# BigCiLeng/bilateral-driving

Hardware: AMD Instinct MI355X
Metric: train iters/sec (fwd+bwd) at 2M Gaussians, 6x1920x1080; HBM roofline % (higher is better)
Workload: dtype f32

## Files before the change

### bilateral_driving_amd/csrc/tiles.hip

```cpp
#include "bds_common.h"
#include "gs_math.h"
#include "scan.h"

namespace bds {

constexpr int kScanBlock = 256;
constexpr int kScanItems = 8;
constexpr int kScanTile = kScanBlock * kScanItems;

__global__ __launch_bounds__(kScanBlock) void scan_reduce_kernel(const uint32_t *__restrict__ in, int64_t n,
                                                                uint32_t *__restrict__ block_sums) {
  __shared__ uint32_t lw[kScanBlock / kWave + 1];
  const int64_t base = (int64_t)blockIdx.x * kScanTile + (int64_t)threadIdx.x * kScanItems;
  uint32_t s = 0;
#pragma unroll
  for (int i = 0; i < kScanItems; i++)
    if (base + i < n) s += in[base + i];
  uint32_t tot;
  block_excl_scan(s, tot, lw);
  if (threadIdx.x == 0) block_sums[blockIdx.x] = tot;
}

__global__ __launch_bounds__(kScanBlock) void scan_small_kernel(uint32_t *__restrict__ data, int64_t n,
                                                               uint64_t *__restrict__ total_out) {
// ... 9 lines not shown
  uint32_t tot;
  uint32_t ex = block_excl_scan(s, tot, lw);
#pragma unroll
  for (int i = 0; i < kScanItems; i++) {
    if (base + i < n) data[base + i] = ex;
    ex += v[i];
  }
  if (total_out && threadIdx.x == 0) *total_out = tot;
}

template <bool kSelfOffset>
__global__ __launch_bounds__(kScanBlock) void scan_apply_kernel(const uint32_t *__restrict__ in, int64_t n,
                                                               const uint32_t *__restrict__ block_offsets,
                                                               uint32_t *__restrict__ out, uint64_t *__restrict__ total_out) {
  __shared__ uint32_t lw[kScanBlock / kWave + 1];
  uint32_t my_offset;
  if (kSelfOffset) {
    uint32_t part = 0;
    for (int b = threadIdx.x; b < (int)blockIdx.x; b += kScanBlock) part += block_offsets[b];
    uint32_t tot;
    block_excl_scan(part, tot, lw);
    my_offset = tot;
  } else {
    my_offset = block_offsets[blockIdx.x];
  }
  const int64_t base = (int64_t)blockIdx.x * kScanTile + (int64_t)threadIdx.x * kScanItems;
  uint32_t v[kScanItems];
  uint32_t s = 0;
#pragma unroll
  for (int i = 0; i < kScanItems; i++) {
    v[i] = base + i < n ? in[base + i] : 0u;
    s += v[i];
  }
  uint32_t tot;
  uint32_t ex = block_excl_scan(s, tot, lw) + my_offset;
#pragma unroll
  for (int i = 0; i < kScanItems; i++) {
    if (base + i < n) out[base + i] = ex;
    ex += v[i];
  }
  if (kSelfOffset && total_out && blockIdx.x == gridDim.x - 1 && threadIdx.x == 0) *total_out = (uint64_t)my_offset + tot;
}

static size_t scan_temp_elems(int64_t n) {
  size_t tot = 0;
  while (n > kScanTile) {
    n = cdiv(n, kScanTile);
    tot += align_up((size_t)n, 4);
  }
  return tot + 4;
}

static int exclusive_scan_u32(const uint32_t *in, uint32_t *out, int64_t n, uint32_t *temp, uint64_t *total_out,
                              hipStream_t st) {
  if (n <= kScanTile) {
    if (in != out) {
      if (hipMemcpyAsync(out, in, sizeof(uint32_t) * n, hipMemcpyDeviceToDevice, st) != hipSuccess) return BDS_ELAUNCH;
    }
    hipLaunchKernelGGL(scan_small_kernel, dim3(1), dim3(kScanBlock), 0, st, out, n, total_out);
    BDS_LAUNCH_CHECK();
    return BDS_OK;
  }
  const int64_t nb = cdiv(n, kScanTile);
  uint32_t *sums = temp;
  hipLaunchKernelGGL(scan_reduce_kernel, dim3((unsigned)nb), dim3(kScanBlock), 0, st, in, n, sums);
  BDS_LAUNCH_CHECK();
  if (nb <= 4096) {
    hipLaunchKernelGGL((scan_apply_kernel<true>), dim3((unsigned)nb), dim3(kScanBlock), 0, st, in, n, sums, out, total_out);
    BDS_LAUNCH_CHECK();
    return BDS_OK;
  }
  int rc = exclusive_scan_u32(sums, sums, nb, temp + align_up((size_t)nb, 4), total_out, st);
  if (rc != BDS_OK) return rc;
  hipLaunchKernelGGL((scan_apply_kernel<false>), dim3((unsigned)nb), dim3(kScanBlock), 0, st, in, n, sums, out, nullptr);
  BDS_LAUNCH_CHECK();
  return BDS_OK;
}

constexpr int kSortBlock = 256;
constexpr int kSortRounds = 16;
constexpr int kSortChunk = kSortBlock * kSortRounds;
constexpr int kSortWaves = kSortBlock / kWave;
constexpr int kGroupShift = 6;

template <int kBins, int kRounds>
__device__ __forceinline__ void chunk_hist(uint32_t *h, const uint32_t *__restrict__ keys, int64_t base, int64_t n, int shift,
                                           uint32_t mask) {
  for (int d = threadIdx.x; d < kBins; d += kSortBlock) h[d] = 0;
  __syncthreads();
#pragma unroll 4
  for (int r = 0; r < kRounds; r++) {
    const int64_t i = base + r * kSortBlock + threadIdx.x;
    if (i < n) atomicAdd(&h[(keys[i] >> shift) & mask], 1u);
  }
  __syncthreads();
}

template <int kRounds, bool kVals>
__device__ __forceinline__ void load_and_count(uint32_t *k, uint32_t *v, const uint32_t *__restrict__ keys_in,
                                               const uint32_t *__restrict__ vals_in, int64_t wbase, int64_t n, int shift, uint32_t mask,
                                               uint32_t *wrow) {
  const int lane = threadIdx.x & (kWave - 1);
#pragma unroll
  for (int r = 0; r < kRounds; r++) {
    const int64_t i = wbase + r * kWave + lane;
    k[r] = 0xFFFFFFFFu;
    if (kVals) v[r] = 0;
    if (i < n) {
      k[r] = keys_in[i];
      if (kVals) v[r] = vals_in[i];
      atomicAdd(&wrow[(k[r] >> shift) & mask], 1u);
    }
  }
}

template <int kBins>
__device__ __forceinline__ void counts_to_positions(uint32_t (&wrun)[kSortWaves][kBins], int d, uint32_t base) {
#pragma unroll
  for (int w = 0; w < kSortWaves; w++) {
    const uint32_t c = wrun[w][d];
    wrun[w][d] = base;
    base += c;
  }
}

template <int kBits = 0>
__device__ __forceinline__ uint32_t rank_round(uint32_t d, bool on, uint32_t *wrow, int bits = kBits) {
  const int lane = threadIdx.x & (kWave - 1);
  const unsigned long long lt = lane == 0 ? 0ull : (~0ull >> (64 - lane));
  unsigned long long peers = __ballot(on);
  auto match_bit = [&](int b) {
    const unsigned long long bal = __ballot((d >> b) & 1u);
    peers &= ((d >> b) & 1u) ? bal : ~bal;
  };
  if constexpr (kBits > 0) {
#pragma unroll
    for (int b = 0; b < kBits; b++) match_bit(b);
  } else {
    for (int b = 0; b < bits; b++) match_bit(b);
  }
  const uint32_t rank = __popcll(peers & lt);
  uint32_t pos = 0;
  if (on) pos = wrow[d];
  __builtin_amdgcn_s_waitcnt(0xc07f);
  __builtin_amdgcn_wave_barrier();
  if (on && rank == 0) wrow[d] = pos + __popcll(peers);
  __builtin_amdgcn_wave_barrier();
  return pos + rank;
}

template <int kPer, int kSums>
__device__ __forceinline__ void grouped_bases(const uint32_t *__restrict__ hist, const uint32_t *__restrict__ ghist, int vb, int nb,
                                              uint32_t (&total)[kPer], uint32_t (&below)[kPer]) {
  constexpr int kBins = kSortBlock * kPer;
  const int ng = (nb + (1 << kGroupShift) - 1) >> kGroupShift, gb = vb >> kGroupShift;
#pragma unroll
  for (int u = 0; u < kPer; u++) { total[u] = 0; below[u] = 0; }
  const uint32_t *gp = ghist + threadIdx.x * kPer;
  int g = 0;
  for (; g + 4 <= ng; g += 4) {
    uint32_t c[4][kPer];
#pragma unroll
    for (int j = 0; j < 4; j++)
#pragma unroll
      for (int u = 0; u < kPer; u++) c[j][u] = gp[(int64_t)(g + j) * kBins + u];
#pragma unroll
    for (int u = 0; u < kPer; u++) {
      total[u] += (c[0][u] + c[1][u]) + (c[2][u] + c[3][u]);
      below[u] += (g < gb ? c[0][u] : 0u) + (g + 1 < gb ? c[1][u] : 0u) + (g + 2 < gb ? c[2][u] : 0u) + (g + 3 < gb ? c[3][u] : 0u);
    }
  }
  for (; g < ng; g++) {
#pragma unroll
    for (int u = 0; u < kPer; u++) {
      const uint32_t c = gp[(int64_t)g * kBins + u];
      total[u] += c;
      if (g < gb) below[u] += c;
    }
  }
  const uint32_t *hp = hist + ((int64_t)gb << kGroupShift) * kBins + threadIdx.x * kPer;
  const int nrows = vb - (gb << kGroupShift);
  uint32_t p[kSums][kPer];
#pragma unroll
  for (int j = 0; j < kSums; j++)
#pragma unroll
    for (int u = 0; u < kPer; u++) p[j][u] = 0;
  int r = 0;
  for (; r + kSums <= nrows; r += kSums) {
    uint32_t a[kSums][kPer];
#pragma unroll
    for (int j = 0; j < kSums; j++)
#pragma unroll
      for (int u = 0; u < kPer; u++) a[j][u] = hp[(int64_t)(r + j) * kBins + u];
#pragma unroll
    for (int j = 0; j < kSums; j++)
#pragma unroll
      for (int u = 0; u < kPer; u++) p[j][u] += a[j][u];
  }
  for (; r < nrows; r++) {
#pragma unroll
    for (int u = 0; u < kPer; u++) p[0][u] += hp[(int64_t)r * kBins + u];
  }
#pragma unroll
  for (int u = 0; u < kPer; u++) {
#pragma unroll
    for (int j = 1; j < kSums; j++) p[0][u] += p[j][u];
    below[u] += p[0][u];
  }
}

template <bool kPairs>
__device__ __forceinline__ void write_out_ordered(const uint32_t *lk, const uint32_t *lv, int cnt, int shift, uint32_t mask,
                                                  const uint32_t *gbase, const uint32_t *dstart, uint32_t *__restrict__ keys_out,
                                                  uint32_t *__restrict__ vals_out, const uint32_t *__restrict__ unpack,
                                                  uint32_t rank_mask) {
  for (int i = threadIdx.x; i < cnt; i += kSortBlock) {
    const uint32_t kk = lk[i];
    const uint32_t d = (kk >> shift) & mask;
    const uint32_t g = gbase[d] + ((uint32_t)i - dstart[d]);
    keys_out[g] = kk;
    if (kPairs) vals_out[g] = lv[i];
    else if (unpack) vals_out[g] = unpack[kk & rank_mask];
  }
}
__device__ __forceinline__ int chunk_count(int64_t n, int64_t bbase) {
  return (int)((n - bbase) < (int64_t)kSortChunk ? (n - bbase) : (int64_t)kSortChunk);
}

__global__ __launch_bounds__(kSortBlock) void radix_hist_kernel(const uint32_t *__restrict__ keys, int64_t n_host,
                                                               const uint64_t *__restrict__ n_dev, int shift,
                                                               uint32_t mask, int nblocks,
                                                               uint32_t *__restrict__ hist ) {
  __shared__ uint32_t h[256];
  chunk_hist<256, kSortRounds>(h, keys, (int64_t)blockIdx.x * kSortChunk, list_length(n_host, n_dev), shift, mask);
  if (threadIdx.x <= mask) hist[(int64_t)threadIdx.x * nblocks + blockIdx.x] = h[threadIdx.x];
}

__global__ __launch_bounds__(kSortBlock) void radix_scatter_lds_kernel(
    const uint32_t *__restrict__ keys_in, const uint32_t *__restrict__ vals_in, int64_t n_host,
    const uint64_t *__restrict__ n_dev, int shift, uint32_t mask, int bits, int nblocks,
    const uint32_t *__restrict__ hist_scanned, uint32_t *__restrict__ keys_out, uint32_t *__restrict__ vals_out) {
  const int64_t n = list_length(n_host, n_dev);
  const int64_t bbase = (int64_t)blockIdx.x * kSortChunk;
  if (bbase >= n) return;
  __shared__ uint32_t wrun[kSortWaves][256];
  __shared__ uint32_t dstart[256], gbase[256];
  __shared__ uint32_t lw[kSortBlock / kWave + 1];
  __shared__ uint32_t lk[kSortChunk], lv[kSortChunk];
  const int tid = threadIdx.x, wv = tid / kWave;
#pragma unroll
  for (int w = 0; w < kSortWaves; w++) wrun[w][tid] = 0;
  __syncthreads();
  const int64_t wbase = bbase + (int64_t)wv * (kSortChunk / kSortWaves);
  uint32_t k[kSortRounds], v[kSortRounds];
  load_and_count<kSortRounds, true>(k, v, keys_in, vals_in, wbase, n, shift, mask, wrun[wv]);
  __syncthreads();
  {
    uint32_t tot = 0;
#pragma unroll
    for (int w = 0; w < kSortWaves; w++) tot += wrun[w][tid];
    uint32_t all;
    const uint32_t base = block_excl_scan(tot, all, lw);
    dstart[tid] = base;
    gbase[tid] = tid <= (int)mask ? hist_scanned[(int64_t)tid * nblocks + blockIdx.x] : 0u;
    counts_to_positions(wrun, tid, base);
  }
  __syncthreads();
#pragma unroll
  for (int r = 0; r < kSortRounds; r++) {
    const bool on = wbase + r * kWave + (tid & (kWave - 1)) < n;
    const uint32_t slot = rank_round((k[r] >> shift) & mask, on, wrun[wv], bits);
    if (on) { lk[slot] = k[r]; lv[slot] = v[r]; }
  }
  __syncthreads();
  write_out_ordered<true>(lk, lv, chunk_count(n, bbase), shift, mask, gbase, dstart, keys_out, vals_out, nullptr, 0u);
}

__global__ __launch_bounds__(kSortBlock) void radix_scatter_keys_kernel(
    const uint32_t *__restrict__ keys_in, int64_t n_host, const uint64_t *__restrict__ n_dev, int shift, uint32_t mask, int bits,
    int nblocks, const uint32_t *__restrict__ hist_scanned, uint32_t *__restrict__ keys_out, const uint32_t *__restrict__ unpack,
    uint32_t rank_mask, uint32_t *__restrict__ vals_out) {
  const int64_t n = list_length(n_host, n_dev);
  const int64_t bbase = (int64_t)blockIdx.x * kSortChunk;
  if (bbase >= n) return;
  __shared__ uint32_t wrun[kSortWaves][256];
  __shared__ uint32_t dstart[256], gbase[256];
  __shared__ uint32_t lw[kSortBlock / kWave + 1];
  __shared__ uint32_t lk[kSortChunk];
  const int tid = threadIdx.x, wv = tid / kWave;
#pragma unroll
  for (int w = 0; w < kSortWaves; w++) wrun[w][tid] = 0;
  __syncthreads();
  const int64_t wbase = bbase + (int64_t)wv * (kSortChunk / kSortWaves);
  uint32_t k[kSortRounds];
  load_and_count<kSortRounds, false>(k, nullptr, keys_in, nullptr, wbase, n, shift, mask, wrun[wv]);
  __syncthreads();
  {
    uint32_t tot = 0;
#pragma unroll
    for (int w = 0; w < kSortWaves; w++) tot += wrun[w][tid];
    uint32_t all;
    const uint32_t base = block_excl_scan(tot, all, lw);
    dstart[tid] = base;
    gbase[tid] = tid <= (int)mask ? hist_scanned[(int64_t)tid * nblocks + blockIdx.x] : 0u;
    counts_to_positions(wrun, tid, base);
  }
  __syncthreads();
#pragma unroll
  for (int r = 0; r < kSortRounds; r++) {
    const bool on = wbase + r * kWave + (tid & (kWave - 1)) < n;
    const uint32_t slot = rank_round((k[r] >> shift) & mask, on, wrun[wv], bits);
    if (on) lk[slot] = k[r];
  }
  __syncthreads();
  write_out_ordered<false>(lk, nullptr, chunk_count(n, bbase), shift, mask, gbase, dstart, keys_out, vals_out, unpack, rank_mask);
}

template <int kBins>
__global__ __launch_bounds__(kSortBlock) void radix_hist_wide_kernel(const uint32_t *__restrict__ keys, int64_t n_host,
                                                                    const uint64_t *__restrict__ n_dev, int shift, uint32_t mask,
                                                                    uint32_t *__restrict__ hist ,
                                                                    uint32_t *__restrict__ ghist ) {
  __shared__ uint32_t h[kBins];
  const int64_t n = list_length(n_host, n_dev), base = (int64_t)blockIdx.x * kSortChunk;
  if (base >= n) return;
  chunk_hist<kBins, kSortRounds>(h, keys, base, n, shift, mask);
  for (int d = threadIdx.x; d < kBins; d += kSortBlock) {
    const uint32_t c = h[d];
    hist[(int64_t)blockIdx.x * kBins + d] = c;
    if (c) atomicAdd(&ghist[(int64_t)(blockIdx.x >> kGroupShift) * kBins + d], c);
  }
}

template <int kBins>
__global__ __launch_bounds__(kSortBlock) void radix_scatter_keys_wide_kernel(
    const uint32_t *__restrict__ keys_in, int64_t n_host, const uint64_t *__restrict__ n_dev, int shift, uint32_t mask, int bits,
    const uint32_t *__restrict__ hist, const uint32_t *__restrict__ ghist, uint32_t *__restrict__ keys_out,
    const uint32_t *__restrict__ unpack, uint32_t rank_mask, uint32_t *__restrict__ vals_out, int32_t *__restrict__ offsets_out,
    int n_offsets) {
  constexpr int kPer = kBins / kSortBlock;
  const int64_t n = list_length(n_host, n_dev);
  const int vb = (int)blockIdx.x;
  const int64_t bbase = (int64_t)vb * kSortChunk;
  if (bbase >= n && !(offsets_out && vb == 0)) return;
  __shared__ uint32_t wrun[kSortWaves][kBins];
  __shared__ uint32_t dstart[kBins], gbase[kBins];
  __shared__ uint32_t lw[kSortBlock / kWave + 1];
  __shared__ uint32_t lk[kSortChunk];
  const int tid = threadIdx.x, wv = tid / kWave;
  for (int d = tid; d < kBins; d += kSortBlock) {
#pragma unroll
    for (int w = 0; w < kSortWaves; w++) wrun[w][d] = 0;
  }
  __syncthreads();
  const int64_t wbase = bbase + (int64_t)wv * (kSortChunk / kSortWaves);
  uint32_t k[kSortRounds];
  load_and_count<kSortRounds, false>(k, nullptr, keys_in, nullptr, wbase, n, shift, mask, wrun[wv]);
  __syncthreads();
  {
    uint32_t tot[kPer], sum = 0;
#pragma unroll
    for (int u = 0; u < kPer; u++) {
      const int d = tid * kPer + u;
      tot[u] = 0;
#pragma unroll
      for (int w = 0; w < kSortWaves; w++) tot[u] += wrun[w][d];
      sum += tot[u];
    }
    uint32_t gt[kPer], below[kPer];
    grouped_bases<kPer, 4>(hist, ghist, vb, (int)((n + kSortChunk - 1) / kSortChunk), gt, below);
    uint32_t gsum = 0;
#pragma unroll
    for (int u = 0; u < kPer; u++) gsum += gt[u];
    uint32_t all;
    uint32_t dbase = block_excl_scan(gsum, all, lw);
    uint32_t base = block_excl_scan(sum, all, lw);
#pragma unroll
    for (int u = 0; u < kPer; u++) {
      const int d = tid * kPer + u;
      dstart[d] = base;
      gbase[d] = dbase + below[u];
      dbase += gt[u];
      if (offsets_out && vb == 0 && d < n_offsets) offsets_out[d] = (int32_t)gbase[d];
      counts_to_positions(wrun, d, base);
      base += tot[u];
    }
  }
  __syncthreads();
#pragma unroll
  for (int r = 0; r < kSortRounds; r++) {
    const bool on = wbase + r * kWave + (tid & (kWave - 1)) < n;
    const uint32_t slot = rank_round((k[r] >> shift) & mask, on, wrun[wv], bits);
    if (on) lk[slot] = k[r];
  }
  __syncthreads();
  write_out_ordered<false>(lk, nullptr, chunk_count(n, bbase), shift, mask, gbase, dstart, keys_out, vals_out, unpack, rank_mask);
}

constexpr int kWideBits = 10;

static size_t radix_temp_elems(int64_t n, int max_bins = 256) {
  const int64_t nblocks = cdiv(n > 0 ? n : 1, kSortChunk);
  const size_t h = align_up((size_t)max_bins * nblocks, 4);
  const size_t group_rows = max_bins > 256 ? (size_t)max_bins * (size_t)cdiv(nblocks, 1 << kGroupShift) : 0;
  const size_t behind = scan_temp_elems((int64_t)max_bins * nblocks);
  return h + (behind > group_rows ? behind : group_rows);
}

static size_t radix_wide_group_elems(int64_t n, int bits) {
  return (size_t)(1 << bits) * (size_t)cdiv(cdiv(n > 0 ? n : 1, kSortChunk), 1 << kGroupShift);
}

static int radix_pass(const uint32_t *kin, const uint32_t *vin, uint32_t *kout, uint32_t *vout, int64_t n, int shift,
                      int bits, uint32_t *temp, hipStream_t st, const uint64_t *n_dev = nullptr) {
  if (n == 0) return BDS_OK;
  const int nblocks = (int)cdiv(n, kSortChunk);
  const uint32_t mask = (1u << bits) - 1u;
  const int64_t hn = (int64_t)(mask + 1) * nblocks;
  uint32_t *hist = temp;
  uint32_t *stemp = temp + align_up((size_t)256 * nblocks, 4);
  hipLaunchKernelGGL(radix_hist_kernel, dim3(nblocks), dim3(kSortBlock), 0, st, kin, n, n_dev, shift, mask, nblocks, hist);
  BDS_LAUNCH_CHECK();
  int rc = exclusive_scan_u32(hist, hist, hn, stemp, nullptr, st);
  if (rc != BDS_OK) return rc;
  hipLaunchKernelGGL(radix_scatter_lds_kernel, dim3(nblocks), dim3(kSortBlock), 0, st, kin, vin, n, n_dev, shift, mask, bits,
                     nblocks, hist, kout, vout);
  BDS_LAUNCH_CHECK();
  return BDS_OK;
}


static int radix_pass_keys(const uint32_t *kin, uint32_t *kout, int64_t n, int shift, int bits, uint32_t *temp, hipStream_t st,
                           const uint32_t *unpack, uint32_t rank_mask, uint32_t *vout, int32_t *offsets_out = nullptr,
                           int n_offsets = 0, const uint64_t *n_dev = nullptr) {
  if (n == 0) return BDS_OK;
  const int nblocks = (int)cdiv(n, kSortChunk);
  const uint32_t mask = (1u << bits) - 1u;
  const int64_t hn = (int64_t)(mask + 1) * nblocks;
  uint32_t *hist = temp;
  uint32_t *stemp = temp + align_up((size_t)(bits > 8 ? (1 << kWideBits) : 256) * nblocks, 4);
  if (bits > 8) {
    uint32_t *ghist = stemp;
    if (bits == 9) {
      hipLaunchKernelGGL((radix_hist_wide_kernel<512>), dim3(nblocks), dim3(kSortBlock), 0, st, kin, n, n_dev, shift, mask, hist, ghist);
      hipLaunchKernelGGL((radix_scatter_keys_wide_kernel<512>), dim3(nblocks), dim3(kSortBlock), 0, st, kin, n, n_dev, shift, mask, bits,
                         hist, ghist, kout, unpack, rank_mask, vout, offsets_out, n_offsets);
    } else {
      hipLaunchKernelGGL((radix_hist_wide_kernel<1024>), dim3(nblocks), dim3(kSortBlock), 0, st, kin, n, n_dev, shift, mask, hist, ghist);
      hipLaunchKernelGGL((radix_scatter_keys_wide_kernel<1024>), dim3(nblocks), dim3(kSortBlock), 0, st, kin, n, n_dev, shift, mask, bits,
                         hist, ghist, kout, unpack, rank_mask, vout, offsets_out, n_offsets);
    }
    BDS_LAUNCH_CHECK();
    return BDS_OK;
  }
  hipLaunchKernelGGL(radix_hist_kernel, dim3(nblocks), dim3(kSortBlock), 0, st, kin, n, n_dev, shift, mask, nblocks, hist);
  BDS_LAUNCH_CHECK();
  int rc = exclusive_scan_u32(hist, hist, hn, stemp, nullptr, st);
  if (rc != BDS_OK) return rc;
  hipLaunchKernelGGL(radix_scatter_keys_kernel, dim3(nblocks), dim3(kSortBlock), 0, st, kin, n, n_dev, shift, mask, bits, nblocks,
                     hist, kout, unpack, rank_mask, vout);
  BDS_LAUNCH_CHECK();
  return BDS_OK;
}

constexpr int kShortRounds = 4;
constexpr int kShortChunk = kSortBlock * kShortRounds;
constexpr int kChunkShift = 10;
static_assert(kShortChunk == (1 << kChunkShift), "chunk shift");
constexpr int64_t kShortSortMax = (int64_t)kShortChunk * 8192;

__device__ __forceinline__ int64_t bounded_count(const uint64_t *n_dev, int64_t n_cap) {
  const int64_t n = (int64_t)*n_dev;
  return (n_cap >= 0 && n > n_cap) ? 0 : n;
}
__global__ __launch_bounds__(kSortBlock) void short_hist_kernel(const uint32_t *__restrict__ keys,
                                                               const uint64_t *__restrict__ n_dev, int64_t n_cap, int shift,
                                                               uint32_t *__restrict__ hist ,
                                                               uint32_t *__restrict__ ghist ) {
  __shared__ uint32_t h[256];
  const int64_t n = bounded_count(n_dev, n_cap), base = (int64_t)blockIdx.x * kShortChunk;
  if (base >= n) return;
  chunk_hist<256, kShortRounds>(h, keys, base, n, shift, 255u);
  const uint32_t c = h[threadIdx.x];
  hist[(int64_t)blockIdx.x * 256 + threadIdx.x] = c;
  if (c) atomicAdd(&ghist[(int64_t)(blockIdx.x >> kGroupShift) * 256 + threadIdx.x], c);
}

__global__ __launch_bounds__(kSortBlock) void short_scatter_kernel(
    const uint32_t *__restrict__ keys_in, const uint32_t *__restrict__ vals_in, const uint64_t *__restrict__ n_dev, int64_t n_cap,
    int shift, const uint32_t *__restrict__ hist, const uint32_t *__restrict__ ghist, uint32_t *__restrict__ keys_out,
    uint32_t *__restrict__ vals_out) {
  const int64_t n = bounded_count(n_dev, n_cap);
  const int vb = (int)blockIdx.x;
  if ((int64_t)vb * kShortChunk >= n) return;
  __shared__ uint32_t wrun[kSortWaves][256];
  __shared__ uint32_t lw[kSortBlock / kWave + 1];
  const int tid = threadIdx.x, wv = tid / kWave;
#pragma unroll
  for (int w = 0; w < kSortWaves; w++) wrun[w][tid] = 0;
  uint32_t total[1], below[1];
  grouped_bases<1, 8>(hist, ghist, vb, (int)((n + kShortChunk - 1) >> kChunkShift), total, below);
  uint32_t all;
  const uint32_t digit_base = block_excl_scan(total[0], all, lw);
  const int64_t wbase = (int64_t)vb * kShortChunk + (int64_t)wv * (kShortChunk / kSortWaves);
  uint32_t k[kShortRounds], v[kShortRounds];
  load_and_count<kShortRounds, true>(k, v, keys_in, vals_in, wbase, n, shift, 255u, wrun[wv]);
  __syncthreads();
  counts_to_positions(wrun, tid, digit_base + below[0]);
  __syncthreads();
#pragma unroll
  for (int r = 0; r < kShortRounds; r++) {
    const bool on = wbase + r * kWave + (tid & (kWave - 1)) < n;
    const uint32_t slot = rank_round<8>((k[r] >> shift) & 255u, on, wrun[wv]);
    if (on) {
      keys_out[slot] = k[r];
      vals_out[slot] = v[r];
    }
  }
}

static size_t short_sort_elems(int64_t n_bound) {
  const int64_t nb = cdiv(n_bound > 0 ? n_bound : 1, kShortChunk), ng = cdiv(nb, 1 << kGroupShift);
  return (size_t)(nb + 4 * ng) * 256;
}

constexpr int kIsectBlock = 256;

__global__ __launch_bounds__(kIsectBlock) void isect_flag_kernel(int64_t CN, const int32_t *__restrict__ radii,
                                                                uint32_t *__restrict__ flags) {
  const int64_t o = (int64_t)blockIdx.x * kIsectBlock + threadIdx.x;
  if (o < CN) flags[o] = radii[o] > 0 ? 1u : 0u;
}

__global__ __launch_bounds__(kIsectBlock) void isect_compact_kernel(int64_t CN, const int32_t *__restrict__ radii,
                                                                   const uint32_t *__restrict__ pos,
                                                                   const float *__restrict__ depths,
                                                                   uint32_t *__restrict__ keys, uint32_t *__restrict__ vals,
                                                                   uint32_t *__restrict__ asc, int compact, int sd) {
  const int64_t o = (int64_t)blockIdx.x * kIsectBlock + threadIdx.x;
  if (o >= CN || radii[o] <= 0) return;
  const uint32_t j = pos[o];
  keys[j] = __float_as_uint(depths[o * sd]);
  vals[j] = compact ? j : (uint32_t)o;
  asc[j] = (uint32_t)o;
}

__global__ __launch_bounds__(kScanBlock) void visible_reduce_kernel(int64_t CN, const int32_t *__restrict__ radii,
                                                                   uint32_t *__restrict__ tile_sums,
                                                                   uint32_t *__restrict__ zero_me, int64_t zero_elems,
                                                                   uint64_t *__restrict__ m_total, int32_t *__restrict__ zero_cn) {
  __shared__ uint32_t lw[kScanBlock / kWave + 1];
  if (blockIdx.x == 0 && threadIdx.x == 0) *m_total = 0;
  for (int64_t i = (int64_t)blockIdx.x * kScanBlock + threadIdx.x; i < zero_elems; i += (int64_t)gridDim.x * kScanBlock)
    zero_me[i] = 0u;
  const int64_t base = (int64_t)blockIdx.x * kScanTile + (int64_t)threadIdx.x * kScanItems;
  uint32_t s = 0;
#pragma unroll
  for (int i = 0; i < kScanItems; i++) {
    if (base + i < CN) {
      s += radii[base + i] > 0 ? 1u : 0u;
      if (zero_cn) zero_cn[base + i] = 0;
    }
  }
  uint32_t tot;
  block_excl_scan(s, tot, lw);
  if (threadIdx.x == 0) tile_sums[blockIdx.x] = tot;
}

constexpr int kCompactSpan = kScanTile / kShortChunk + 1;
__global__ __launch_bounds__(kScanBlock) void visible_compact_kernel(int64_t CN, const int32_t *__restrict__ radii,
                                                                    const float *__restrict__ depths,
                                                                    const uint32_t *__restrict__ tile_sums,
                                                                    uint32_t *__restrict__ keys, uint32_t *__restrict__ vals,
                                                                    uint32_t *__restrict__ hist, uint32_t *__restrict__ ghist,
                                                                    uint64_t *__restrict__ n_vis_out, uint32_t *__restrict__ asc,
                                                                    int compact, int sums_per_tile, int sd) {
  constexpr int kSpan = kCompactSpan;
  __shared__ uint32_t lw[kScanBlock / kWave + 1];
  __shared__ uint32_t h[kSpan][256];
  const int vb = (int)blockIdx.x, nvb = (int)gridDim.x;
  uint32_t part = 0;
  for (int b = threadIdx.x; b < vb * sums_per_tile; b += kScanBlock) part += tile_sums[b];
  uint32_t my_offset;
  block_excl_scan(part, my_offset, lw);
  const uint32_t per_sum = (uint32_t)(kScanTile / sums_per_tile);
  const int n_sums = (int)(((uint32_t)CN + per_sum - 1u) / per_sum);
  uint32_t own = 0;
  for (int k = 0; k < sums_per_tile; k++) {
    const int b = vb * sums_per_tile + k;
    if (b < n_sums) own += tile_sums[b];
  }
  if (own == 0) {
    if (vb == nvb - 1 && threadIdx.x == 0) *n_vis_out = (uint64_t)my_offset;
    return;
  }
#pragma unroll
  for (int t = 0; t < kSpan; t++) h[t][threadIdx.x] = 0;
  const int64_t base = (int64_t)vb * kScanTile + (int64_t)threadIdx.x * kScanItems;
  bool vis[kScanItems];
  uint32_t s = 0;
#pragma unroll
  for (int i = 0; i < kScanItems; i++) {
    vis[i] = base + i < CN && radii[base + i] > 0;
    s += vis[i] ? 1u : 0u;
  }
  uint32_t tot;
  uint32_t j = block_excl_scan(s, tot, lw) + my_offset;
  const uint32_t chunk0 = my_offset >> kChunkShift;
#pragma unroll
  for (int i = 0; i < kScanItems; i++) {
    if (vis[i]) {
      const uint32_t key = __float_as_uint(depths[(base + i) * sd]);
      keys[j] = key;
      vals[j] = compact ? j : (uint32_t)(base + i);
      asc[j] = (uint32_t)(base + i);
      atomicAdd(&h[(j >> kChunkShift) - chunk0][key & 255u], 1u);
      j++;
    }
  }
  __syncthreads();
#pragma unroll
  for (int t = 0; t < kSpan; t++) {
    const uint32_t c = h[t][threadIdx.x];
    if (c) {
      atomicAdd(&hist[(int64_t)(chunk0 + t) * 256 + threadIdx.x], c);
      atomicAdd(&ghist[(int64_t)((chunk0 + t) >> kGroupShift) * 256 + threadIdx.x], c);
    }
  }
  if (vb == nvb - 1 && threadIdx.x == 0) *n_vis_out = (uint64_t)my_offset + tot;
}

struct RowStage {
  float mx[kIsectBlock], my[kIsectBlock], a[kIsectBlock], b[kIsectBlock], c[kIsectBlock], qmax[kIsectBlock];
  int x0[kIsectBlock], x1[kIsectBlock], y0[kIsectBlock];
  uint32_t id[kIsectBlock];
  uint32_t cam_base[kIsectBlock];
  uint32_t rowoff[kIsectBlock + 1];
  uint32_t lw[kIsectBlock / kWave + 1];
};

constexpr int kRecWords = 12;

__device__ __forceinline__ uint32_t stage_rows(RowStage &S, int64_t j0, int64_t n_vis, int64_t N, const uint32_t *__restrict__ sorted_idx,
                                               const uint32_t *__restrict__ asc ,
                                               const float *__restrict__ means2d, const int32_t *__restrict__ radii,
                                               const float *__restrict__ conics, const float *__restrict__ opacities,
                                               int tile_size, int tile_w, int tile_h, float4 *__restrict__ rec_out,
                                               const float4 *__restrict__ rec_in, const ProjLayout pl) {
  const int t = threadIdx.x;
  const int64_t j = j0 + t;
  uint32_t nrows = 0;
  if (j < n_vis) {
    if (rec_in != nullptr) {
      const float4 r0 = rec_in[j * 3], r1 = rec_in[j * 3 + 1], r2 = rec_in[j * 3 + 2];
      nrows = __float_as_uint(r2.y);
      S.mx[t] = r0.x; S.my[t] = r0.y; S.a[t] = r0.z; S.b[t] = r0.w;
      S.c[t] = r1.x; S.qmax[t] = r1.y; S.x0[t] = __float_as_int(r1.z); S.x1[t] = __float_as_int(r1.w);
      S.y0[t] = __float_as_int(r2.x); S.id[t] = __float_as_uint(r2.z); S.cam_base[t] = __float_as_uint(r2.w);
    } else {
      const uint32_t val = sorted_idx[j];
      const uint32_t o = asc ? asc[val] : val;
      const int r = proj_radius(pl, means2d, radii, (int64_t)o);
      float mx = means2d[(int64_t)o * pl.s2], my = means2d[(int64_t)o * pl.s2 + 1];
      float a = 0.f, b = 0.f, c = 0.f, q_max = 0.f, op = 0.f;
      if (conics != nullptr) {
        a = conics[(int64_t)o * pl.sc]; b = conics[(int64_t)o * pl.sc + 1]; c = conics[(int64_t)o * pl.sc + 2];
        op = opacities[(int64_t)o * pl.so];
      }
      int x0 = 0, y0 = 0, x1 = 0, y1 = 0;
      if (r > 0) {
        bool ok;
        if (conics == nullptr) {
          tile_rect(mx, my, r, tile_size, tile_w, tile_h, x0, y0, x1, y1);
          ok = x1 > x0 && y1 > y0;
        } else {
          ok = tile_rect_tight(mx, my, r, a, b, c, op, tile_size, tile_w, tile_h, x0, y0, x1, y1, q_max);
        }
        if (ok) nrows = (uint32_t)(y1 - y0);
      } else {
        mx = my = a = b = c = 0.f;
      }
      const uint32_t cam_base = (int64_t)o < N ? 0u : (uint32_t)((uint32_t)o / (uint32_t)N) * (uint32_t)(tile_w * tile_h);
      S.mx[t] = mx; S.my[t] = my; S.a[t] = a; S.b[t] = b; S.c[t] = c; S.qmax[t] = q_max;
      S.x0[t] = x0; S.x1[t] = x1; S.y0[t] = y0; S.id[t] = val; S.cam_base[t] = cam_base;
      if (rec_out != nullptr) {
        rec_out[j * 3] = make_float4(mx, my, a, b);
        rec_out[j * 3 + 1] = make_float4(c, q_max, __int_as_float(x0), __int_as_float(x1));
        rec_out[j * 3 + 2] = make_float4(__int_as_float(y0), __uint_as_float(nrows), __uint_as_float(val), __uint_as_float(cam_base));
      }
    }
  }
  uint32_t total;
  const uint32_t ex = block_excl_scan(nrows, total, S.lw);
  S.rowoff[t] = ex;
  if (t == 0) S.rowoff[kIsectBlock] = total;
  __syncthreads();
  return total;
}

__device__ __forceinline__ int row_owner(const RowStage &S, uint32_t r) {
  int lo = 0, hi = kIsectBlock;
#pragma unroll
  for (int s = 0; s < 8; s++) {
    const int mid = (lo + hi) >> 1;
    if (S.rowoff[mid] <= r) lo = mid; else hi = mid;
  }
  return lo;
}

// ... 196 lines not shown
  return BDS_OK;
}

extern "C" size_t bds_isect_visible_ids_offset(int C, int64_t N) {
  if (C < 1 || N < 0) return 0;
  char *const base = reinterpret_cast<char *>(static_cast<uintptr_t>(4096));
  const PrepWs L = prep_layout(base, (int64_t)C * N);
  return static_cast<size_t>(reinterpret_cast<char *>(L.asc) - base);
}

extern "C" size_t bds_isect_block_counts_offset(int C, int64_t N) {
  if (C < 1 || N < 0) return 0;
  char *const base = reinterpret_cast<char *>(static_cast<uintptr_t>(4096));
  const PrepWs L = prep_layout(base, (int64_t)C * N);
  return static_cast<size_t>(reinterpret_cast<char *>(L.temp) - base);
}

extern "C" size_t bds_isect_prepare_workspace_bytes(int C, int64_t N) {
  if (C < 1 || N < 0) return 0;
  return prep_layout(nullptr, (int64_t)C * N).bytes;
}

extern "C" size_t bds_isect_build_workspace_bytes(int C, int64_t N, int64_t M) {
  (void)C; (void)N;
  if (M < 0) return 0;
  return build_layout(nullptr, M).bytes;
}

constexpr int kCountMEff = 2, kCountVisEff = 3, kCountOverflow = 4;
__global__ __launch_bounds__(256) void finish_counts_kernel(const uint32_t *__restrict__ btot, int nblocks, uint64_t *__restrict__ counts_dev,
                                                           volatile int64_t *__restrict__ counts_host, int64_t cap_m, int64_t cap_vis) {
  __shared__ unsigned long long part[256];
  unsigned long long s0 = 0, s1 = 0, s2 = 0, s3 = 0;
  int b = threadIdx.x;
  for (; b + 768 < nblocks; b += 1024) {
    const uint32_t a0 = btot[b], a1 = btot[b + 256], a2 = btot[b + 512], a3 = btot[b + 768];
    s0 += a0; s1 += a1; s2 += a2; s3 += a3;
  }
  for (; b < nblocks; b += 256) s0 += btot[b];
  part[threadIdx.x] = (s0 + s1) + (s2 + s3);
  __syncthreads();
  for (int o = 128; o > 0; o >>= 1) {
    if ((int)threadIdx.x < o) part[threadIdx.x] += part[threadIdx.x + o];
    __syncthreads();
  }
  if (threadIdx.x == 0) {
    counts_dev[0] = part[0];
    const uint64_t nv = counts_dev[1];
    if (cap_m >= 0) {
      const bool over = (int64_t)part[0] > cap_m || (int64_t)nv > cap_vis;
      counts_dev[kCountMEff] = over ? 0ull : part[0];
      counts_dev[kCountVisEff] = over ? 0ull : nv;
      counts_dev[kCountOverflow] = over ? 1ull : 0ull;
      if (counts_host && over) counts_host[2] = 1;
    }
    if (counts_host) { counts_host[0] = (int64_t)part[0]; counts_host[1] = (int64_t)nv; }
  }
  if (counts_host) __threadfence_system();
}

static int prepare_enqueue(int C, int64_t N, const float *means2d, const int32_t *radii, const float *depths,
                           const float *conics, const float *opacities, int tile_size, int tile_w, int tile_h,
                           int32_t *tiles_per_gauss, void *ws, size_t ws_bytes, int compact, bds_stream_t stream,
                           uint64_t **counts_dev, const uint32_t **btot_out, int *nblocks_out, int64_t nvis_bound = -1) {
  BDS_REQUIRE(C >= 1 && N >= 0 && tile_size > 0 && tile_w > 0 && tile_h > 0);
  const int64_t CN = (int64_t)C * N;
  BDS_REQUIRE(CN < (int64_t)1 << 31);
  BDS_REQUIRE((int64_t)C * tile_w * tile_h < (int64_t)1 << 31);
  *counts_dev = nullptr;
  *btot_out = nullptr; *nblocks_out = 0;
  if (CN == 0) return BDS_OK;
  BDS_REQUIRE(means2d && radii && depths && ws);
  BDS_REQUIRE((conics == nullptr) == (opacities == nullptr));
  const ProjLayout pl = proj_layout(means2d, depths, conics, opacities);
  PrepWs L = prep_layout(ws, CN);
  if (ws_bytes < L.bytes) return BDS_EWORKSPACE;
  hipStream_t st = as_stream(stream);
  if (nvis_bound < 0 || nvis_bound > CN || !option_get(kOptCapLaunch)) nvis_bound = CN;
  const int64_t n_cap = nvis_bound < CN ? nvis_bound : (int64_t)-1;
  const unsigned grid = (unsigned)cdiv(nvis_bound > 0 ? nvis_bound : 1, kIsectBlock);
  uint64_t *n_vis = L.total + 1;
  int rc;
  if (CN <= kShortSortMax && option_get(kOptShortSort)) {
    const int64_t nb = cdiv(CN, kShortChunk), ng = cdiv(nb, 1 << kGroupShift);
    const unsigned nb_launch = (unsigned)cdiv(nvis_bound > 0 ? nvis_bound : 1, kShortChunk);
    uint32_t *hist = L.tables, *ghist = L.tables + nb * 256;
    const unsigned tiles = (unsigned)cdiv(CN, kScanTile);
    if (!(compact & 2))
      hipLaunchKernelGGL(visible_reduce_kernel, dim3(tiles), dim3(kScanBlock), 0, st, CN, radii, L.temp, L.tables,
                         (int64_t)short_sort_elems(CN), L.total, tiles_per_gauss);
    hipLaunchKernelGGL(visible_compact_kernel, dim3(tiles), dim3(kScanBlock), 0, st, CN, radii, depths, L.temp, L.ka, L.va, hist,
                       ghist, n_vis, L.asc, compact & 1, (compact & 2) ? kScanTile / 256 : 1, pl.sd);
    BDS_LAUNCH_CHECK();
    uint32_t *kin = L.ka, *vin = L.va, *kout = L.kb, *vout = L.vb;
    for (int p = 0; p < 4; p++) {
      uint32_t *gh = ghist + (int64_t)p * ng * 256;
      if (p > 0) hipLaunchKernelGGL(short_hist_kernel, dim3(nb_launch), dim3(kSortBlock), 0, st, kin, n_vis, n_cap, 8 * p, hist, gh);
      hipLaunchKernelGGL(short_scatter_kernel, dim3(nb_launch), dim3(kSortBlock), 0, st, kin, vin, n_vis, n_cap, 8 * p, hist, gh, kout,
                         vout);
      uint32_t *t;
      t = kin; kin = kout; kout = t;
      t = vin; vin = vout; vout = t;
    }
    BDS_LAUNCH_CHECK();
    hipLaunchKernelGGL(isect_count_rows_kernel, dim3(grid), dim3(kIsectBlock), 0, st, n_vis, n_cap, L.va, means2d, radii, conics,
                       opacities, tile_size, tile_w, tile_h, tiles_per_gauss, N, L.rec, L.btot,
                       (compact & 1) ? L.asc : (const uint32_t *)nullptr, pl);
    BDS_LAUNCH_CHECK();
  } else {
    BDS_REQUIRE(!(compact & 2));
    if (hipMemsetAsync(L.total, 0, sizeof(uint64_t), st) != hipSuccess) return BDS_ELAUNCH;
    hipLaunchKernelGGL(isect_flag_kernel, dim3(grid), dim3(kIsectBlock), 0, st, CN, radii, L.kb);
    BDS_LAUNCH_CHECK();
    rc = exclusive_scan_u32(L.kb, L.cum, CN, L.temp, n_vis, st);
    if (rc != BDS_OK) return rc;
    hipLaunchKernelGGL(isect_compact_kernel, dim3(grid), dim3(kIsectBlock), 0, st, CN, radii, L.cum, depths, L.ka, L.va, L.asc, compact, pl.sd);
    BDS_LAUNCH_CHECK();
    uint32_t *kin = L.ka, *vin = L.va, *kout = L.kb, *vout = L.vb;
    for (int p = 0; p < 4; p++) {
      rc = radix_pass(kin, vin, kout, vout, CN, 8 * p, 8, L.temp, st, n_vis);
      if (rc != BDS_OK) return rc;
      uint32_t *t;
      t = kin; kin = kout; kout = t;
      t = vin; vin = vout; vout = t;
    }
    if (tiles_per_gauss && hipMemsetAsync(tiles_per_gauss, 0, sizeof(int32_t) * CN, st) != hipSuccess) return BDS_ELAUNCH;
    hipLaunchKernelGGL(isect_count_rows_kernel, dim3(grid), dim3(kIsectBlock), 0, st, n_vis, (int64_t)-1, L.va, means2d, radii, conics,
                       opacities, tile_size, tile_w, tile_h, tiles_per_gauss, N, L.rec, L.btot,
                       compact ? L.asc : (const uint32_t *)nullptr, pl);
    BDS_LAUNCH_CHECK();
  }
  (void)rc;
  *counts_dev = L.total;
  *btot_out = L.btot; *nblocks_out = (int)grid;
  return BDS_OK;
}

extern "C" int bds_isect_prepare(int C, int64_t N, const float *means2d, const int32_t *radii, const float *depths,
                                 const float *conics, const float *opacities, int tile_size, int tile_w, int tile_h,
                                 int32_t *tiles_per_gauss, void *ws, size_t ws_bytes, int64_t M_capacity, int64_t n_visible_capacity,
                                 int64_t *counts, void *event, int compact, bds_stream_t stream) {
  BDS_REQUIRE((M_capacity < 0) == (n_visible_capacity < 0));
  const bool dev = M_capacity >= 0, sync = !dev && !event;
  if (dev) {
    BDS_REQUIRE(!event && (int64_t)C * N > 0);
  } else {
    BDS_REQUIRE(counts);
    counts[0] = 0; counts[1] = 0;
  }
  uint64_t *counts_dev = nullptr;
  const uint32_t *btot = nullptr;
  int nblocks = 0;
  int rc = prepare_enqueue(C, N, means2d, radii, depths, conics, opacities, tile_size, tile_w, tile_h, tiles_per_gauss, ws, ws_bytes,
                           compact, stream, &counts_dev, &btot, &nblocks, dev ? n_visible_capacity : (int64_t)-1);
  if (rc != BDS_OK) return rc;
  hipStream_t st = as_stream(stream);
  if (counts_dev != nullptr) {
    void *mapped = nullptr;
    if (!sync && counts && hipHostGetDevicePointer(&mapped, counts, 0) != hipSuccess) {
      (void)hipGetLastError();
      if (dev) return BDS_EINVAL;
      mapped = nullptr;
    }
    hipLaunchKernelGGL(finish_counts_kernel, dim3(1), dim3(256), 0, st, btot, nblocks, counts_dev, static_cast<volatile int64_t *>(mapped),
                       M_capacity, n_visible_capacity);
    BDS_LAUNCH_CHECK();
    if (!dev && mapped == nullptr &&
        hipMemcpyAsync(counts, counts_dev, 2 * sizeof(uint64_t), hipMemcpyDeviceToHost, st) != hipSuccess)
      return BDS_ELAUNCH;
    if (sync && hipStreamSynchronize(st) != hipSuccess) return BDS_ELAUNCH;
  }
  if (event && hipEventRecord(static_cast<hipEvent_t>(event), st) != hipSuccess) return BDS_ELAUNCH;
  return BDS_OK;
}

extern "C" size_t bds_isect_counts_offset(int which) {
  return (which >= 0 && which <= kCountOverflow) ? (size_t)which * sizeof(uint64_t) : (size_t)0;
}

extern "C" int bds_isect_build(int C, int64_t N, int64_t M, int64_t n_visible, const float *means2d, const int32_t *radii,
                               const float *depths, const float *conics, const float *opacities, int tile_size,
                               int tile_w, int tile_h, const void *ws,
// ... 117 lines not shown
```

Baseline: 1137.

## Add sub-group histogram level to bound per-block radix prefix reads

Adds a third histogram level (groups of 8 chunks) filled by extra atomics in the hist and compact kernels. The scatter kernels then compute their digit base from group totals, at most 7 sub-group rows and at most 7 own-chunk rows. These rows are fetched with fixed-count, fully unrolled buffer loads, replacing a variable-length loop over up to 63 rows. In the wide scatter kernel the base computation also moves ahead of the key loading so its latency can overlap. The cost is extra atomics and workspace, and the workspace layout offsets change.

Measured after the change: 1150 (median of 6 runs). 1.01x the previous value.

```diff
diff --git a/bilateral_driving_amd/csrc/tiles.hip b/bilateral_driving_amd/csrc/tiles.hip
--- a/bilateral_driving_amd/csrc/tiles.hip
+++ b/bilateral_driving_amd/csrc/tiles.hip
@@ -115,6 +115,7 @@
 constexpr int kSortChunk = kSortBlock * kSortRounds;
 constexpr int kSortWaves = kSortBlock / kWave;
 constexpr int kGroupShift = 6;
+constexpr int kSubShift = 3;
 
 template <int kBins, int kRounds>
 __device__ __forceinline__ void chunk_hist(uint32_t *h, const uint32_t *__restrict__ keys, int64_t base, int64_t n, int shift,
@@ -182,63 +183,73 @@
   return pos + rank;
 }
 
-template <int kPer, int kSums>
-__device__ __forceinline__ void grouped_bases(const uint32_t *__restrict__ hist, const uint32_t *__restrict__ ghist, int vb, int nb,
-                                              uint32_t (&total)[kPer], uint32_t (&below)[kPer]) {
+struct RowTable {
+  __amdgpu_buffer_rsrc_t rsrc;
+  __device__ __forceinline__ RowTable(const uint32_t *base, int rows, int bins)
+      : rsrc(__builtin_amdgcn_make_buffer_rsrc(const_cast<uint32_t *>(base), 0, rows * bins * (int)sizeof(uint32_t), 0x00020000)) {}
+  __device__ __forceinline__ uint32_t load(int row_bytes, uint32_t col_bytes) const {
+    return __builtin_amdgcn_raw_buffer_load_b32(rsrc, (int)col_bytes, row_bytes, 0);
+  }
+};
+
+template <int kPer>
+__device__ __forceinline__ void grouped_bases(const uint32_t *__restrict__ hist, const uint32_t *__restrict__ ghist,
+                                              const uint32_t *__restrict__ shist, int vb, int nb, uint32_t (&total)[kPer],
+                                              uint32_t (&below)[kPer]) {
   constexpr int kBins = kSortBlock * kPer;
-  const int ng = (nb + (1 << kGroupShift) - 1) >> kGroupShift, gb = vb >> kGroupShift;
+  constexpr int kSubRows = (1 << (kGroupShift - kSubShift)) - 1, kOwnRows = (1 << kSubShift) - 1;
+  const int ng = (nb + (1 << kGroupShift) - 1) >> kGroupShift, gb = vb >> kGroupShift, sb = vb >> kSubShift;
+  const int n_sub = sb - (gb << (kGroupShift - kSubShift)), n_own = vb - (sb << kSubShift);
+  constexpr int kRowBytes = kBins * (int)sizeof(uint32_t);
+  const uint32_t col = threadIdx.x * kPer;
+  const RowTable sp(shist + ((int64_t)gb << (kGroupShift - kSubShift)) * kBins, kSubRows, kBins);
+  const RowTable hp(hist + ((int64_t)sb << kSubShift) * kBins, kOwnRows, kBins);
+  uint32_t cs[kSubRows][kPer], ch[kOwnRows][kPer];
+#pragma unroll
+  for (int j = 0; j < kSubRows; j++)
+#pragma unroll
+    for (int u = 0; u < kPer; u++) cs[j][u] = sp.load((j < n_sub ? j : 0) * kRowBytes, (col + u) * (uint32_t)sizeof(uint32_t));
+#pragma unroll
+  for (int j = 0; j < kOwnRows; j++)
+#pragma unroll
+    for (int u = 0; u < kPer; u++) ch[j][u] = hp.load((j < n_own ? j : 0) * kRowBytes, (col + u) * (uint32_t)sizeof(uint32_t));
 #pragma unroll
   for (int u = 0; u < kPer; u++) { total[u] = 0; below[u] = 0; }
-  const uint32_t *gp = ghist + threadIdx.x * kPer;
   int g = 0;
   for (; g + 4 <= ng; g += 4) {
     uint32_t c[4][kPer];
 #pragma unroll
     for (int j = 0; j < 4; j++)
 #pragma unroll
-      for (int u = 0; u < kPer; u++) c[j][u] = gp[(int64_t)(g + j) * kBins + u];
+      for (int u = 0; u < kPer; u++) c[j][u] = (ghist + (int64_t)(g + j) * kBins)[col + u];
 #pragma unroll
     for (int u = 0; u < kPer; u++) {
       total[u] += (c[0][u] + c[1][u]) + (c[2][u] + c[3][u]);
       below[u] += (g < gb ? c[0][u] : 0u) + (g + 1 < gb ? c[1][u] : 0u) + (g + 2 < gb ? c[2][u] : 0u) + (g + 3 < gb ? c[3][u] : 0u);
     }
   }
-  for (; g < ng; g++) {
-#pragma unroll
-    for (int u = 0; u < kPer; u++) {
-      const uint32_t c = gp[(int64_t)g * kBins + u];
-      total[u] += c;
-      if (g < gb) below[u] += c;
-    }
-  }
-  const uint32_t *hp = hist + ((int64_t)gb << kGroupShift) * kBins + threadIdx.x * kPer;
-  const int nrows = vb - (gb << kGroupShift);
-  uint32_t p[kSums][kPer];
-#pragma unroll
-  for (int j = 0; j < kSums; j++)
-#pragma unroll
-    for (int u = 0; u < kPer; u++) p[j][u] = 0;
-  int r = 0;
-  for (; r + kSums <= nrows; r += kSums) {
-    uint32_t a[kSums][kPer];
-#pragma unroll
-    for (int j = 0; j < kSums; j++)
-#pragma unroll
-      for (int u = 0; u < kPer; u++) a[j][u] = hp[(int64_t)(r + j) * kBins + u];
-#pragma unroll
-    for (int j = 0; j < kSums; j++)
-#pragma unroll
-      for (int u = 0; u < kPer; u++) p[j][u] += a[j][u];
-  }
-  for (; r < nrows; r++) {
-#pragma unroll
-    for (int u = 0; u < kPer; u++) p[0][u] += hp[(int64_t)r * kBins + u];
+  {
+    uint32_t c[3][kPer];
+#pragma unroll
+    for (int j = 0; j < 3; j++)
+#pragma unroll
+      for (int u = 0; u < kPer; u++) c[j][u] = (ghist + (int64_t)(g + j < ng ? g + j : 0) * kBins)[col + u];
+#pragma unroll
+    for (int j = 0; j < 3; j++)
+#pragma unroll
+      for (int u = 0; u < kPer; u++) {
+        total[u] += g + j < ng ? c[j][u] : 0u;
+        below[u] += g + j < gb ? c[j][u] : 0u;
+      }
   }
 #pragma unroll
   for (int u = 0; u < kPer; u++) {
-#pragma unroll
-    for (int j = 1; j < kSums; j++) p[0][u] += p[j][u];
-    below[u] += p[0][u];
+    uint32_t s = 0;
+#pragma unroll
+    for (int j = 0; j < kSubRows; j++) s += j < n_sub ? cs[j][u] : 0u;
+#pragma unroll
+    for (int j = 0; j < kOwnRows; j++) s += j < n_own ? ch[j][u] : 0u;
+    below[u] += s;
   }
 }
 
@@ -353,7 +364,8 @@
 __global__ __launch_bounds__(kSortBlock) void radix_hist_wide_kernel(const uint32_t *__restrict__ keys, int64_t n_host,
                                                                     const uint64_t *__restrict__ n_dev, int shift, uint32_t mask,
                                                                     uint32_t *__restrict__ hist ,
-                                                                    uint32_t *__restrict__ ghist ) {
+                                                                    uint32_t *__restrict__ ghist ,
+                                                                    uint32_t *__restrict__ shist ) {
   __shared__ uint32_t h[kBins];
   const int64_t n = list_length(n_host, n_dev), base = (int64_t)blockIdx.x * kSortChunk;
   if (base >= n) return;
@@ -361,15 +373,19 @@
   for (int d = threadIdx.x; d < kBins; d += kSortBlock) {
     const uint32_t c = h[d];
     hist[(int64_t)blockIdx.x * kBins + d] = c;
-    if (c) atomicAdd(&ghist[(int64_t)(blockIdx.x >> kGroupShift) * kBins + d], c);
+    if (c) {
+      atomicAdd(&ghist[(int64_t)(blockIdx.x >> kGroupShift) * kBins + d], c);
+      atomicAdd(&shist[(int64_t)(blockIdx.x >> kSubShift) * kBins + d], c);
+    }
   }
 }
 
 template <int kBins>
 __global__ __launch_bounds__(kSortBlock) void radix_scatter_keys_wide_kernel(
     const uint32_t *__restrict__ keys_in, int64_t n_host, const uint64_t *__restrict__ n_dev, int shift, uint32_t mask, int bits,
-    const uint32_t *__restrict__ hist, const uint32_t *__restrict__ ghist, uint32_t *__restrict__ keys_out,
-    const uint32_t *__restrict__ unpack, uint32_t rank_mask, uint32_t *__restrict__ vals_out, int32_t *__restrict__ offsets_out,
+    const uint32_t *__restrict__ hist, const uint32_t *__restrict__ ghist, const uint32_t *__restrict__ shist,
+    uint32_t *__restrict__ keys_out, const uint32_t *__restrict__ unpack, uint32_t rank_mask, uint32_t *__restrict__ vals_out,
+    int32_t *__restrict__ offsets_out,
     int n_offsets) {
   constexpr int kPer = kBins / kSortBlock;
   const int64_t n = list_length(n_host, n_dev);
@@ -385,6 +401,15 @@
 #pragma unroll
     for (int w = 0; w < kSortWaves; w++) wrun[w][d] = 0;
   }
+  {
+    uint32_t gt[kPer], below[kPer];
+    grouped_bases<kPer>(hist, ghist, shist, vb, (int)((n + kSortChunk - 1) / kSortChunk), gt, below);
+#pragma unroll
+    for (int u = 0; u < kPer; u++) {
+      dstart[tid * kPer + u] = gt[u];
+      gbase[tid * kPer + u] = below[u];
+    }
+  }
   __syncthreads();
   const int64_t wbase = bbase + (int64_t)wv * (kSortChunk / kSortWaves);
   uint32_t k[kSortRounds];
@@ -400,11 +425,13 @@
       for (int w = 0; w < kSortWaves; w++) tot[u] += wrun[w][d];
       sum += tot[u];
     }
-    uint32_t gt[kPer], below[kPer];
-    grouped_bases<kPer, 4>(hist, ghist, vb, (int)((n + kSortChunk - 1) / kSortChunk), gt, below);
-    uint32_t gsum = 0;
-#pragma unroll
-    for (int u = 0; u < kPer; u++) gsum += gt[u];
+    uint32_t gt[kPer], below[kPer], gsum = 0;
+#pragma unroll
+    for (int u = 0; u < kPer; u++) {
+      gt[u] = dstart[tid * kPer + u];
+      below[u] = gbase[tid * kPer + u];
+      gsum += gt[u];
+    }
     uint32_t all;
     uint32_t dbase = block_excl_scan(gsum, all, lw);
     uint32_t base = block_excl_scan(sum, all, lw);
@@ -432,16 +459,18 @@
 
 constexpr int kWideBits = 10;
 
+static int64_t partial_rows(int64_t nb) { return cdiv(nb, 1 << kGroupShift) + cdiv(nb, 1 << kSubShift); }
+
 static size_t radix_temp_elems(int64_t n, int max_bins = 256) {
   const int64_t nblocks = cdiv(n > 0 ? n : 1, kSortChunk);
   const size_t h = align_up((size_t)max_bins * nblocks, 4);
-  const size_t group_rows = max_bins > 256 ? (size_t)max_bins * (size_t)cdiv(nblocks, 1 << kGroupShift) : 0;
+  const size_t group_rows = max_bins > 256 ? (size_t)max_bins * (size_t)partial_rows(nblocks) : 0;
   const size_t behind = scan_temp_elems((int64_t)max_bins * nblocks);
   return h + (behind > group_rows ? behind : group_rows);
 }
 
 static size_t radix_wide_group_elems(int64_t n, int bits) {
-  return (size_t)(1 << bits) * (size_t)cdiv(cdiv(n > 0 ? n : 1, kSortChunk), 1 << kGroupShift);
+  return (size_t)(1 << bits) * (size_t)partial_rows(cdiv(n > 0 ? n : 1, kSortChunk));
 }
 
 static int radix_pass(const uint32_t *kin, const uint32_t *vin, uint32_t *kout, uint32_t *vout, int64_t n, int shift,
@@ -473,15 +502,15 @@
   uint32_t *hist = temp;
   uint32_t *stemp = temp + align_up((size_t)(bits > 8 ? (1 << kWideBits) : 256) * nblocks, 4);
   if (bits > 8) {
-    uint32_t *ghist = stemp;
+    uint32_t *ghist = stemp, *shist = stemp + (size_t)(1 << bits) * (size_t)cdiv(nblocks, 1 << kGroupShift);
     if (bits == 9) {
-      hipLaunchKernelGGL((radix_hist_wide_kernel<512>), dim3(nblocks), dim3(kSortBlock), 0, st, kin, n, n_dev, shift, mask, hist, ghist);
+      hipLaunchKernelGGL((radix_hist_wide_kernel<512>), dim3(nblocks), dim3(kSortBlock), 0, st, kin, n, n_dev, shift, mask, hist, ghist, shist);
       hipLaunchKernelGGL((radix_scatter_keys_wide_kernel<512>), dim3(nblocks), dim3(kSortBlock), 0, st, kin, n, n_dev, shift, mask, bits,
-                         hist, ghist, kout, unpack, rank_mask, vout, offsets_out, n_offsets);
+                         hist, ghist, shist, kout, unpack, rank_mask, vout, offsets_out, n_offsets);
     } else {
-      hipLaunchKernelGGL((radix_hist_wide_kernel<1024>), dim3(nblocks), dim3(kSortBlock), 0, st, kin, n, n_dev, shift, mask, hist, ghist);
+      hipLaunchKernelGGL((radix_hist_wide_kernel<1024>), dim3(nblocks), dim3(kSortBlock), 0, st, kin, n, n_dev, shift, mask, hist, ghist, shist);
       hipLaunchKernelGGL((radix_scatter_keys_wide_kernel<1024>), dim3(nblocks), dim3(kSortBlock), 0, st, kin, n, n_dev, shift, mask, bits,
-                         hist, ghist, kout, unpack, rank_mask, vout, offsets_out, n_offsets);
+                         hist, ghist, shist, kout, unpack, rank_mask, vout, offsets_out, n_offsets);
     }
     BDS_LAUNCH_CHECK();
     return BDS_OK;
@@ -509,20 +538,24 @@
 __global__ __launch_bounds__(kSortBlock) void short_hist_kernel(const uint32_t *__restrict__ keys,
                                                                const uint64_t *__restrict__ n_dev, int64_t n_cap, int shift,
                                                                uint32_t *__restrict__ hist ,
-                                                               uint32_t *__restrict__ ghist ) {
+                                                               uint32_t *__restrict__ ghist ,
+                                                               uint32_t *__restrict__ shist ) {
   __shared__ uint32_t h[256];
   const int64_t n = bounded_count(n_dev, n_cap), base = (int64_t)blockIdx.x * kShortChunk;
   if (base >= n) return;
   chunk_hist<256, kShortRounds>(h, keys, base, n, shift, 255u);
   const uint32_t c = h[threadIdx.x];
   hist[(int64_t)blockIdx.x * 256 + threadIdx.x] = c;
-  if (c) atomicAdd(&ghist[(int64_t)(blockIdx.x >> kGroupShift) * 256 + threadIdx.x], c);
+  if (c) {
+    atomicAdd(&ghist[(int64_t)(blockIdx.x >> kGroupShift) * 256 + threadIdx.x], c);
+    atomicAdd(&shist[(int64_t)(blockIdx.x >> kSubShift) * 256 + threadIdx.x], c);
+  }
 }
 
 __global__ __launch_bounds__(kSortBlock) void short_scatter_kernel(
     const uint32_t *__restrict__ keys_in, const uint32_t *__restrict__ vals_in, const uint64_t *__restrict__ n_dev, int64_t n_cap,
-    int shift, const uint32_t *__restrict__ hist, const uint32_t *__restrict__ ghist, uint32_t *__restrict__ keys_out,
-    uint32_t *__restrict__ vals_out) {
+    int shift, const uint32_t *__restrict__ hist, const uint32_t *__restrict__ ghist, const uint32_t *__restrict__ shist,
+    uint32_t *__restrict__ keys_out, uint32_t *__restrict__ vals_out) {
   const int64_t n = bounded_count(n_dev, n_cap);
   const int vb = (int)blockIdx.x;
   if ((int64_t)vb * kShortChunk >= n) return;
@@ -532,7 +565,7 @@
 #pragma unroll
   for (int w = 0; w < kSortWaves; w++) wrun[w][tid] = 0;
   uint32_t total[1], below[1];
-  grouped_bases<1, 8>(hist, ghist, vb, (int)((n + kShortChunk - 1) >> kChunkShift), total, below);
+  grouped_bases<1>(hist, ghist, shist, vb, (int)((n + kShortChunk - 1) >> kChunkShift), total, below);
   uint32_t all;
   const uint32_t digit_base = block_excl_scan(total[0], all, lw);
   const int64_t wbase = (int64_t)vb * kShortChunk + (int64_t)wv * (kShortChunk / kSortWaves);
@@ -553,8 +586,8 @@
 }
 
 static size_t short_sort_elems(int64_t n_bound) {
-  const int64_t nb = cdiv(n_bound > 0 ? n_bound : 1, kShortChunk), ng = cdiv(nb, 1 << kGroupShift);
-  return (size_t)(nb + 4 * ng) * 256;
+  const int64_t nb = cdiv(n_bound > 0 ? n_bound : 1, kShortChunk);
+  return (size_t)(nb + 4 * partial_rows(nb)) * 256;
 }
 
 constexpr int kIsectBlock = 256;
@@ -606,7 +639,7 @@
                                                                     const uint32_t *__restrict__ tile_sums,
                                                                     uint32_t *__restrict__ keys, uint32_t *__restrict__ vals,
                                                                     uint32_t *__restrict__ hist, uint32_t *__restrict__ ghist,
-                                                                    uint64_t *__restrict__ n_vis_out, uint32_t *__restrict__ asc,
+                                                                    uint32_t *__restrict__ shist, uint64_t *__restrict__ n_vis_out, uint32_t *__restrict__ asc,
                                                                     int compact, int sums_per_tile, int sd) {
   constexpr int kSpan = kCompactSpan;
   __shared__ uint32_t lw[kScanBlock / kWave + 1];
@@ -658,6 +691,7 @@
     if (c) {
       atomicAdd(&hist[(int64_t)(chunk0 + t) * 256 + threadIdx.x], c);
       atomicAdd(&ghist[(int64_t)((chunk0 + t) >> kGroupShift) * 256 + threadIdx.x], c);
+      atomicAdd(&shist[(int64_t)((chunk0 + t) >> kSubShift) * 256 + threadIdx.x], c);
     }
   }
   if (vb == nvb - 1 && threadIdx.x == 0) *n_vis_out = (uint64_t)my_offset + tot;
@@ -1020,7 +1054,7 @@
   uint64_t *n_vis = L.total + 1;
   int rc;
   if (CN <= kShortSortMax && option_get(kOptShortSort)) {
-    const int64_t nb = cdiv(CN, kShortChunk), ng = cdiv(nb, 1 << kGroupShift);
+    const int64_t nb = cdiv(CN, kShortChunk), ng = cdiv(nb, 1 << kGroupShift), npr = partial_rows(nb);
     const unsigned nb_launch = (unsigned)cdiv(nvis_bound > 0 ? nvis_bound : 1, kShortChunk);
     uint32_t *hist = L.tables, *ghist = L.tables + nb * 256;
     const unsigned tiles = (unsigned)cdiv(CN, kScanTile);
@@ -1028,14 +1062,14 @@
       hipLaunchKernelGGL(visible_reduce_kernel, dim3(tiles), dim3(kScanBlock), 0, st, CN, radii, L.temp, L.tables,
                          (int64_t)short_sort_elems(CN), L.total, tiles_per_gauss);
     hipLaunchKernelGGL(visible_compact_kernel, dim3(tiles), dim3(kScanBlock), 0, st, CN, radii, depths, L.temp, L.ka, L.va, hist,
-                       ghist, n_vis, L.asc, compact & 1, (compact & 2) ? kScanTile / 256 : 1, pl.sd);
+                       ghist, ghist + ng * 256, n_vis, L.asc, compact & 1, (compact & 2) ? kScanTile / 256 : 1, pl.sd);
     BDS_LAUNCH_CHECK();
     uint32_t *kin = L.ka, *vin = L.va, *kout = L.kb, *vout = L.vb;
     for (int p = 0; p < 4; p++) {
-      uint32_t *gh = ghist + (int64_t)p * ng * 256;
-      if (p > 0) hipLaunchKernelGGL(short_hist_kernel, dim3(nb_launch), dim3(kSortBlock), 0, st, kin, n_vis, n_cap, 8 * p, hist, gh);
-      hipLaunchKernelGGL(short_scatter_kernel, dim3(nb_launch), dim3(kSortBlock), 0, st, kin, vin, n_vis, n_cap, 8 * p, hist, gh, kout,
-                         vout);
+      uint32_t *gh = ghist + (int64_t)p * npr * 256, *sh = gh + ng * 256;
+      if (p > 0) hipLaunchKernelGGL(short_hist_kernel, dim3(nb_launch), dim3(kSortBlock), 0, st, kin, n_vis, n_cap, 8 * p, hist, gh, sh);
+      hipLaunchKernelGGL(short_scatter_kernel, dim3(nb_launch), dim3(kSortBlock), 0, st, kin, vin, n_vis, n_cap, 8 * p, hist, gh, sh,
+                         kout, vout);
       uint32_t *t;
       t = kin; kin = kout; kout = t;
       t = vin; vin = vout; vout = t;
```
